# seqan/lambda

Hardware: AMD Instinct MI355X
Metric: GCUPS (gapped extension, full-rectangle parity mode; pass-1 cells per second of whole step) searchp BLOSUM62 (higher is better)
Workload: dtype f16x2 (exact small integers) + int32

## Files before the change

lambda_amd/csrc/lx_score_f16.hip:

```cpp
#include <hip/hip_runtime.h>

#include "lx_aids.h"
#include "lx_dp_common.h"

namespace lx
{

typedef _Float16 h2 __attribute__((ext_vector_type(2)));

#ifndef LX_F16_UNROLL
#define LX_F16_UNROLL 2
#endif
#ifndef LX_F16_CKPT_WAVES
#define LX_F16_CKPT_WAVES 3
#endif
#define LX_PRAGMA(x) _Pragma(#x)
#define LX_UNROLL(n) LX_PRAGMA(unroll n)

__device__ __forceinline__ h2 hmax3(h2 a, h2 b, h2 c)
{
    return __builtin_elementwise_maximum(__builtin_elementwise_maximum(a, b), c);
}
__device__ __forceinline__ h2 hmax(h2 a, h2 b)
{
    return __builtin_elementwise_maximum(a, b);
}
__device__ __forceinline__ h2 hsplat(float x)
{
    return h2{(_Float16)x, (_Float16)x};
}
__device__ __forceinline__ h2 as_h2(uint32_t x)
{
    return __builtin_bit_cast(h2, x);
}
__device__ __forceinline__ uint32_t as_u32(h2 x)
{
    return __builtin_bit_cast(uint32_t, x);
}

constexpr uint32_t kHalfNegInf2 = 0xfc00fc00u;

constexpr uint32_t kHalfTwoPowMinus24x2 = 0x00010001u;
__device__ __forceinline__ uint32_t c16_pack(h2 value_scaled, h2 diff_scaled)
{
    return (as_u32(diff_scaled) << 11) | as_u32(value_scaled);
}

template <int G, int C>
struct PairGeo
{
    static constexpr int kGroups   = 64 / G;
    static constexpr int kPanel    = G * C;
    static constexpr int kUsedDw   = (C + 1) / 2;
    static constexpr int kLaneDw   = (kUsedDw + 3) & ~3;
    static constexpr int kRowDw    = kLaneDw * G;
};

template <int G, int C, bool CKPT>
__global__ __launch_bounds__(64, (CKPT ? (C > 19 ? 2 : LX_F16_CKPT_WAVES) : 1)) void score_pair_kernel(ScoreParams p)
{
    static_assert(C <= 32, "profile rows hold 32 halves per lane");
    using Geo = PairGeo<G, C>;
    extern __shared__ uint32_t lds[];

    int const  lane     = threadIdx.x;
    int const  grp      = lane / G;
    int const  g        = lane % G;
    bool const is_first = (g == 0);

    uint64_t const pair   = (uint64_t)blockIdx.x * Geo::kGroups + grp;
    uint64_t const eA     = 2 * pair, eB = 2 * pair + 1;
    bool const     actA   = eA < p.n, actB = eB < p.n;

    ScoringDev const * __restrict__ sc = p.sc;
    int const      ge    = sc->ge;
    int const      nrows = p.nrows;
    uint32_t const padt  = (uint32_t)(nrows - 1);

    int             lq = 0, lsA = 0, lsB = 0;
    uint8_t const * q  = p.q_res;
    uint8_t const * sA = p.s_res;
    uint8_t const * sB = p.s_res;
    uint64_t        q_off = 0;
    if (actA)
    {
        Extension const x = p.ext[eA];
        lq    = (int)x.q_len;
        q_off = x.q_off;
        q += x.q_off;
        lsA = (int)x.s_len;
        if (lsA != 0)
            sA += x.s_off;
    }
    uint64_t q_offB = q_off;
    int      lqB    = lq;
    if (actB)
    {
        Extension const x = p.ext[eB];
        lqB    = (int)x.q_len;
        q_offB = x.q_off;
        lsB    = (int)x.s_len;
        if (lsB != 0)
            sB += x.s_off;
    }
    int const share_g = (p.pair_share > 0 && p.pair_share < Geo::kGroups) ? p.pair_share : Geo::kGroups;
    int const blk     = grp / share_g;
    {
        int const      leader = blk * share_g * G;
        uint64_t const q0     = ((uint64_t)(uint32_t)__shfl((int)(q_off >> 32), leader) << 32) | (uint32_t)__shfl((int)(uint32_t)q_off, leader);
        int const      l0     = __shfl(lq, leader);
        bool const     lead_in = __shfl(actA ? 1 : 0, leader) != 0;
        if (lead_in && ((actA && (q_off != q0 || lq != l0)) || (actB && (q_offB != q0 || lqB != l0))))
            atomicExch(p.err, 2);
    }

    int ls_max = max(lsA, lsB);
    int ls_min = min(actA ? lsA : 0x7fffffff, actB ? lsB : 0x7fffffff);
#pragma unroll
    for (int off = 32; off >= 1; off >>= 1)
    {
        ls_max = max(ls_max, __shfl_xor(ls_max, off));
        ls_min = min(ls_min, __shfl_xor(ls_min, off));
    }
    ls_max = __builtin_amdgcn_readfirstlane(ls_max);
    ls_min = __builtin_amdgcn_readfirstlane(ls_min);
    int const steps = (ls_max + G - 1 + 3) & ~3;

    int const col0  = g * C;
    int       bound = lq * sc->smax;
    if (__ballot(bound + (-ge) * (steps + G + 2) + sc->smax + 2 > 2046) != 0)
    {
        bound = 0;
#pragma unroll
        for (int c = 0; c < C; ++c)
        {
            int const j = col0 + c;
            if (j < lq)
                bound += sc->rowmax[q[j] & (kAlph - 1)];
        }
#pragma unroll
        for (int off = G / 2; off >= 1; off >>= 1)
            bound += __shfl_xor(bound, off);
    }
    bool too_big = __ballot((lq > Geo::kPanel) || (bound + (-ge) * (steps + G + 2) + sc->smax + 2 > 2046)) != 0;
    if constexpr (CKPT)
    {
        bool const broken = (__ballot(lq > Geo::kPanel) != 0) || (uint32_t)steps > p.steps_cap;
        if (broken && lane == 0)
            atomicExch(p.err, 3);
        too_big = too_big || broken;
    }

    if (too_big)
    {
        if (is_first)
        {
            if (actA)
                p.out_score[eA] = -1;
            if (actB)
                p.out_score[eB] = -1;
            if constexpr (CKPT)
            {
                EndCell none{};
                none.score = -1;
                if (actA)
                    p.ends[eA] = none;
                if (actB)
                    p.ends[eB] = none;
            }
        }
        return;
    }

    int const slot_dw = blk * (nrows * Geo::kRowDw);
    if (grp % share_g == 0)
    {
#pragma unroll 1
        for (int d = 0; d < Geo::kUsedDw; ++d)
        {
            uint32_t rows[2][16];
#pragma unroll
            for (int cc = 0; cc < 2; ++cc)
            {
                int const c  = 2 * d + cc;
                int const j  = col0 + c;
                uint32_t  ql = kAlph - 1;
                if (c < C && j < lq)
                    ql = q[j] & (kAlph - 1);
                uint4 const * mrow = reinterpret_cast<uint4 const *>(sc->mat_h + ql * kAlph);
#pragma unroll
                for (int x = 0; x < 4; ++x)
                {
                    uint4 const v      = mrow[x];
                    rows[cc][4 * x + 0] = v.x;
                    rows[cc][4 * x + 1] = v.y;
                    rows[cc][4 * x + 2] = v.z;
                    rows[cc][4 * x + 3] = v.w;
                }
            }
            uint32_t * dst = lds + slot_dw + g * Geo::kLaneDw + d;
#pragma unroll
            for (int w = 0; w < 16; ++w)
            {
                if (2 * w < nrows)
                {
                    dst[(2 * w) * Geo::kRowDw]     = __builtin_amdgcn_perm(rows[1][w], rows[0][w], 0x05040100u);
                    dst[(2 * w + 1) * Geo::kRowDw] = __builtin_amdgcn_perm(rows[1][w], rows[0][w], 0x07060302u);
                }
            }
        }
    }
    __builtin_amdgcn_fence(__ATOMIC_RELEASE, "wavefront");
    __builtin_amdgcn_wave_barrier();

    uint32_t const row_base  = (uint32_t)(slot_dw + g * Geo::kLaneDw) * 4u;
    constexpr uint32_t kRowBytes = Geo::kRowDw * 4;

    h2 const GE = hsplat((float)ge), G2 = hsplat((float)sc->g2), NGE = hsplat((float)-ge);
    h2       Z  = hsplat((float)(ge * g));
    h2       Hrow[C], F0[C];
#pragma unroll
    for (int c = 0; c < C; ++c)
    {
        Hrow[c] = Z + GE;
        F0[c]   = Z;
    }
    h2 diag0 = Z + GE;
    h2 sendH = Z + GE;
    h2 sendE = as_h2(kHalfNegInf2);
    h2 best  = hsplat(0.f);
    int      rowA = 0, rowB = 0;
    uint32_t tie  = 0;
    h2 const C24 = as_h2(kHalfTwoPowMinus24x2), NC24 = -C24, GEc = GE * C24;
    h2       nZc = -(Z * C24);
    h2       cmax = as_h2(kHalfNegInf2);
    using Lay = Ckpt16Layout<G, C>;
    constexpr uint32_t kW       = 2 * Geo::kGroups;
    constexpr bool     wslots   = CKPT;
    uint32_t * const   waveBase = CKPT ? p.ckpt + (uint64_t)blockIdx.x * kW * p.ckpt_stride : nullptr;
    uint32_t * const   slotA    = !CKPT ? nullptr : wslots ? waveBase + (2 * grp) * (G * 4) : p.ckpt + (actA ? eA : p.n) * p.ckpt_stride;
    uint32_t * const   slotB    = !CKPT ? nullptr : wslots ? waveBase + (2 * grp + 1) * (G * 4) : p.ckpt + (actB ? eB : p.n) * p.ckpt_stride;
    uint32_t const     octMul   = wslots ? kW * G : G;
    uint32_t const     ckMul    = (wslots ? kW * G : G) * (Lay::kCkDw / 4);
    uint32_t * const stage = lds + ((Geo::kGroups + share_g - 1) / share_g) * (nrows * Geo::kRowDw) + lane;

    auto step = [&](uint32_t tA, uint32_t tB, int slot8)
    {
        uint4 const * ra = reinterpret_cast<uint4 const *>(reinterpret_cast<char const *>(lds) + row_base + tA * kRowBytes);
        uint4 const * rb = reinterpret_cast<uint4 const *>(reinterpret_cast<char const *>(lds) + row_base + tB * kRowBytes);
        uint32_t      pa[Geo::kLaneDw], pb[Geo::kLaneDw];
#pragma unroll
        for (int x = 0; x < (Geo::kUsedDw + 3) / 4; ++x)
        {
            if (4 * x + 2 >= Geo::kUsedDw)
            {
                uint2 const va = *reinterpret_cast<uint2 const *>(ra + x), vb = *reinterpret_cast<uint2 const *>(rb + x);
                pa[4 * x] = va.x; pa[4 * x + 1] = va.y;
                pb[4 * x] = vb.x; pb[4 * x + 1] = vb.y;
            }
            else
            {
                uint4 const va = ra[x], vb = rb[x];
                pa[4 * x] = va.x; pa[4 * x + 1] = va.y; pa[4 * x + 2] = va.z; pa[4 * x + 3] = va.w;
                pb[4 * x] = vb.x; pb[4 * x + 1] = vb.y; pb[4 * x + 2] = vb.z; pb[4 * x + 3] = vb.w;
            }
        }

        h2 const recvH = as_h2((uint32_t)shift_from_left<G>((int)as_u32(sendH), (int)as_u32(Z), is_first));
        h2       Ecur  = as_h2((uint32_t)shift_from_left<G>((int)as_u32(sendE), (int)kHalfNegInf2, is_first));
        h2       dg    = diag0;
        diag0          = recvH;

        h2 const ZN     = Z + NGE;
        h2       rowmax = as_h2(kHalfNegInf2);
        h2       h      = Z;
#pragma unroll
        for (int c = 0; c < C; ++c)
        {
            uint32_t const sel = (c & 1) ? 0x07060302u : 0x05040100u;
            h2 const       sub = as_h2(__builtin_amdgcn_perm(pb[c >> 1], pa[c >> 1], sel));
            h2 const       tt  = dg + sub;
            dg                 = Hrow[c];
            h                  = hmax3(tt, Ecur, F0[c]);
            h2 const A         = h + G2;
            F0[c]              = hmax3(F0[c], A, ZN);
            Ecur               = hmax(Ecur, A) + GE;
            Hrow[c]            = h;
            if (c & 1)
                rowmax = hmax3(rowmax, Hrow[c - 1], h);
        }
        if (C & 1)
            rowmax = hmax(rowmax, h);
        sendH = h;
        sendE = Ecur;
        h2 const cand = rowmax - Z;
        if constexpr (CKPT)
        {
            cmax = hmax(cmax, cand);
            h2 const hc           = h * C24;
            stage[slot8 * 64]     = c16_pack(hc + nZc, __builtin_elementwise_fma(Ecur, NC24, hc));
            nZc                   = nZc + GEc;
        }
        else
            best = hmax(best, cand);
        Z = ZN;
    };
    auto flush_codes = [&](int k0)
    {
        if constexpr (CKPT)
        {
            uint32_t cw[8];
#pragma unroll
            for (int u = 0; u < 8; ++u)
                cw[u] = stage[u * 64];
            uint32_t const oi = ((uint32_t)k0 / 8) * octMul + (uint32_t)g;
            reinterpret_cast<uint4 *>(slotA)[oi] = make_uint4(__builtin_amdgcn_perm(cw[1], cw[0], 0x05040100u), __builtin_amdgcn_perm(cw[3], cw[2], 0x05040100u),
                                                              __builtin_amdgcn_perm(cw[5], cw[4], 0x05040100u), __builtin_amdgcn_perm(cw[7], cw[6], 0x05040100u));
            reinterpret_cast<uint4 *>(slotB)[oi] = make_uint4(__builtin_amdgcn_perm(cw[1], cw[0], 0x07060302u), __builtin_amdgcn_perm(cw[3], cw[2], 0x07060302u),
                                                              __builtin_amdgcn_perm(cw[5], cw[4], 0x07060302u), __builtin_amdgcn_perm(cw[7], cw[6], 0x07060302u));
        }
    };
    auto book = [&](int k0)
    {
        if constexpr (CKPT)
        {
            h2 const       nb   = hmax(best, cmax);
            uint32_t const rose = as_u32(nb) ^ as_u32(best), met = as_u32(cmax) ^ as_u32(best);
            bool const     gtA = (rose & 0xffffu) != 0, gtB = (rose >> 16) != 0;
            bool const     eqA = (met & 0xffffu) == 0, eqB = (met >> 16) == 0;
            int const last = k0 + 3 - g;
            rowA = gtA ? last : rowA;
            rowB = gtB ? last : rowB;
            tie  = (gtA ? (tie & ~1u) : (tie | (eqA ? 1u : 0u)));
            tie  = (gtB ? (tie & ~2u) : (tie | (eqB ? 2u : 0u)));
            best = nb;
            cmax = as_h2(kHalfNegInf2);
        }
    };
    auto chunk_done = [&](int k0)
    {
        if constexpr (CKPT)
        {
#ifndef LX_EXP_NO_FLUSH
            if (k0 & 4)
                flush_codes(k0);
#endif
        }
    };
    auto rowck_store = [&](int k0)
    {
        if constexpr (CKPT)
        {
            h2 const nzic = nZc - GEc, nGEc = -GEc;
            uint32_t code[2 * Lay::kCkDw];
#pragma unroll
            for (int c = 0; c < 2 * Lay::kCkDw; ++c)
                code[c] = c < C ? c16_pack(__builtin_elementwise_fma(Hrow[c < C ? c : 0], C24, nzic),
                                           __builtin_elementwise_fma(Hrow[c < C ? c : 0] - F0[c < C ? c : 0], C24, nGEc))
                                : 0u;
            uint32_t const base0 = (uint32_t)(Lay::bnd_dwords(p.steps_cap) / 4);
            uint4 * const  dA = wslots ? reinterpret_cast<uint4 *>(waveBase) + kW * base0 + (2 * grp) * (G * (Lay::kCkDw / 4)) : reinterpret_cast<uint4 *>(slotA) + base0;
            uint4 * const  dB = wslots ? reinterpret_cast<uint4 *>(waveBase) + kW * base0 + (2 * grp + 1) * (G * (Lay::kCkDw / 4)) : reinterpret_cast<uint4 *>(slotB) + base0;
#pragma unroll
            for (int x = 0; x < Lay::kCkDw / 4; ++x)
            {
                uint32_t wa[4], wb[4];
#pragma unroll
                for (int b = 0; b < 4; ++b)
                {
                    int const c = 2 * (4 * x + b);
                    wa[b]       = __builtin_amdgcn_perm(code[c + 1], code[c], 0x05040100u);
                    wb[b]       = __builtin_amdgcn_perm(code[c + 1], code[c], 0x07060302u);
                }
                uint32_t const qi = ((uint32_t)(k0 + 3) / 16) * ckMul + (uint32_t)g * (Lay::kCkDw / 4) + (uint32_t)x;
                dA[qi] = make_uint4(wa[0], wa[1], wa[2], wa[3]);
                dB[qi] = make_uint4(wb[0], wb[1], wb[2], wb[3]);
            }
        }
    };

    uint32_t const lscA = (uint32_t)max(lsA, 1) - 1u, lscB = (uint32_t)max(lsB, 1) - 1u;
    auto fetch_checked = [&](int k0, uint32_t (&ta)[4], uint32_t (&tb)[4])
    {
#pragma unroll
        for (int u = 0; u < 4; ++u)
        {
            uint32_t const i = (uint32_t)(k0 + u - g);
            ta[u]            = sA[min(i, lscA)];
            tb[u]            = sB[min(i, lscB)];
        }
    };
    auto mask_checked = [&](int k0, uint32_t (&ta)[4], uint32_t (&tb)[4])
    {
#pragma unroll
        for (int u = 0; u < 4; ++u)
        {
            uint32_t const i = (uint32_t)(k0 + u - g);
            ta[u]            = (i < (uint32_t)lsA) ? (ta[u] & (kAlph - 1)) : padt;
            tb[u]            = (i < (uint32_t)lsB) ? (tb[u] & (kAlph - 1)) : padt;
        }
    };

    int const steady_lo = (G - 1 + 3) & ~3;
    int const steady_hi = ls_min - 3;
    uint8_t const * spA = sA - g;
    uint8_t const * spB = sB - g;

    auto chunk_stores = [&](int k0)
    {
        chunk_done(k0);
        if (((k0 + 4) & 15) == 0)
        {
            book(k0);
#ifndef LX_EXP_NO_ROWCK
            rowck_store(k0);
#endif
        }
    };
    int      k0 = 0;
    uint32_t na[4], nb[4];
    fetch_checked(0, na, nb);
    while (k0 < steps)
    {
        bool const cur_steady = (k0 >= steady_lo) && (k0 < steady_hi);
        if (!cur_steady)
        {
            uint32_t ca[4] = {na[0], na[1], na[2], na[3]}, cb[4] = {nb[0], nb[1], nb[2], nb[3]};
            mask_checked(k0, ca, cb);
            fetch_checked(k0 + 4, na, nb);
#pragma unroll 1
            for (int u = 0; u < 4; ++u)
                step(ca[u], cb[u], (k0 & 4) + u);
            if constexpr (CKPT)
                asm volatile("" : "+v"(na[0]), "+v"(na[1]), "+v"(na[2]), "+v"(na[3]), "+v"(nb[0]), "+v"(nb[1]), "+v"(nb[2]), "+v"(nb[3])::"memory");
            chunk_stores(k0);
            k0 += 4;
        }
        else
        {
            uint32_t wa = *reinterpret_cast<unaligned_u32 const *>(spA + k0);
            uint32_t wb = *reinterpret_cast<unaligned_u32 const *>(spB + k0);
            if constexpr (CKPT)
                asm volatile("" : "+v"(wa), "+v"(wb)::"memory");
            while (k0 < steady_hi)
            {
                uint32_t const ca = wa, cb = wb;
                int const      kn = max(min(k0 + 4, ls_min - 4), 0);
                wa                = *reinterpret_cast<unaligned_u32 const *>(spA + kn);
                wb                = *reinterpret_cast<unaligned_u32 const *>(spB + kn);
LX_UNROLL(LX_F16_UNROLL)
                for (int u = 0; u < 4; ++u)
                    step((ca >> (8 * u)) & (kAlph - 1), (cb >> (8 * u)) & (kAlph - 1), (k0 & 4) + u);
                if constexpr (CKPT)
                    asm volatile("" : "+v"(wa), "+v"(wb)::"memory");
                chunk_stores(k0);
                k0 += 4;
            }
            fetch_checked(k0, na, nb);
        }
    }
    if (steps & 4)
        flush_codes(steps);
    if (steps & 15)
        book(steps - 4);

    if constexpr (!CKPT)
    {
#pragma unroll
        for (int off = G / 2; off >= 1; off >>= 1)
            best = hmax(best, as_h2((uint32_t)__shfl_xor((int)as_u32(best), off)));

        if (is_first)
        {
            if (actA)
                p.out_score[eA] = (int)(float)best.x;
            if (actB)
                p.out_score[eB] = (int)(float)best.y;
        }
    }
    else
    {
        auto finish = [&](int lbest, int lrow, int ltie, bool act, uint64_t e)
        {
            int gbest = lbest, gstrip = g, grow = lrow, gtie = ltie;
#pragma unroll
            for (int off = 1; off < G; off <<= 1)
            {
                int const  ob = __shfl_xor(gbest, off), os = __shfl_xor(gstrip, off), orow = __shfl_xor(grow, off), ot = __shfl_xor(gtie, off);
                bool const take = ob > gbest || (ob == gbest && os < gstrip);
                gbest  = take ? ob : gbest;
                gstrip = take ? os : gstrip;
                grow   = take ? orow : grow;
                gtie   = take ? ot : gtie;
            }
            if (is_first && act)
            {
                EndCell ec{};
                if (gbest > 0)
                {
                    ec.score = gbest;
                    ec.q_end = -(gstrip + 1);
                    ec.s_end = grow + 1;
                    ec.flags = (gtie ? kEndAmbiguous : 0) | kEndCompact | kEndWaveSlots;
                }
                p.ends[e]      = ec;
                p.out_score[e] = gbest;
            }
        };
        finish((int)(float)best.x, rowA, (int)(tie & 1u), actA, eA);
        finish((int)(float)best.y, rowB, (int)((tie >> 1) & 1u), actB, eB);
    }
}

template <int G, int C, bool CKPT = false>
static hipError_t launch_pair_cfg(ScoreParams const & p, hipStream_t stream)
{
    using Geo = PairGeo<G, C>;
    uint64_t const per_wave = 2ull * Geo::kGroups;
    uint64_t const blocks   = (p.n + per_wave - 1) / per_wave;
    if (blocks > 0x7fffffffull)
        return hipErrorInvalidValue;
    int const    slots = (p.pair_share > 0 && p.pair_share < Geo::kGroups) ? Geo::kGroups / p.pair_share : 1;
    if (slots * p.pair_share != Geo::kGroups && slots != 1)
        return hipErrorInvalidValue;
    size_t const lds = ((size_t)slots * (size_t)p.nrows * Geo::kRowDw + (CKPT ? 64 * 8 : 0)) * sizeof(uint32_t);
    hipLaunchKernelGGL((score_pair_kernel<G, C, CKPT>), dim3((unsigned)blocks), dim3(64), lds, stream, p);
    return hipGetLastError();
}

hipError_t launch_score_pair(int cfg, ScoreParams const & p, hipStream_t stream)
{
    if (p.n == 0)
        return hipSuccess;
    if (p.ckpt)
    {
        if (!p.ends || p.steps_cap % 16 != 0)
            return hipErrorInvalidValue;
        return cfg == 0   ? launch_pair_cfg<8, 19, true>(p, stream)
               : cfg == 5 ? launch_pair_cfg<16, 13, true>(p, stream)
               : cfg == 1 ? launch_pair_cfg<8, 13, true>(p, stream)
               : cfg == 7 ? launch_pair_cfg<8, 25, true>(p, stream)
                          : hipErrorInvalidValue;
    }
    switch (cfg)
    {
        case 0: return launch_pair_cfg<8, 19>(p, stream);
        case 1: return launch_pair_cfg<8, 13>(p, stream);
        case 2: return launch_pair_cfg<8, 16>(p, stream);
        case 3: return launch_pair_cfg<8, 8>(p, stream);
        case 4: return launch_pair_cfg<8, 24>(p, stream);
        case 5: return launch_pair_cfg<16, 13>(p, stream);
        case 6: return launch_pair_cfg<16, 10>(p, stream);
        case 7: return launch_pair_cfg<8, 25>(p, stream);
        default: return hipErrorInvalidValue;
    }
}

int score_pair_cfg_for(uint32_t max_qlen)
{
    if (max_qlen <= 64)
        return 3;
    if (max_qlen <= 104)
        return 1;
    if (max_qlen <= 128)
        return 2;
    if (max_qlen <= 152)
        return 0;
    if (max_qlen <= 192)
        return 4;
    if (max_qlen <= 200)
        return 7;
    if (max_qlen <= 208)
        return 5;
    return -1;
}

int score_pair_cfg_for_runs_of_8(uint32_t max_qlen)
{
    if (max_qlen <= 160)
        return 6;
    if (max_qlen <= 208)
        return 5;
    return -1;
}

int score_pair_cfg_cols(int cfg)
{
    static int const c[8] = {19, 13, 16, 8, 24, 13, 10, 25};
    return (cfg >= 0 && cfg < 8) ? c[cfg] : 0;
}

int score_pair_cfg_group(int cfg) { return (cfg == 5 || cfg == 6) ? 16 : 8; }

size_t score_pair_profile_bytes(int cfg, int nrows)
{
    int const G = score_pair_cfg_group(cfg), C = score_pair_cfg_cols(cfg);
    return (size_t)nrows * (size_t)((((C + 1) / 2 + 3) & ~3) * G) * sizeof(uint32_t);
}

}
```

Before: 5927.

## Interleave lane groups for DPP row shifts and share profile building across group

Remaps lanes so that for G=8 two groups interleave within each 16-lane DPP row. The left-neighbour H/E handoff can then use a single update_dpp row_shr instead of the shuffle-based shift_from_left, and reductions use strided xor shuffles. The LDS query-profile build is now split across all lanes of the sharing block rather than done by the leader group alone. This shortens the per-cell inner-loop dependency and the prologue, at the cost of more complex lane indexing. It risks subtle correctness issues in the handling of the boundary lane.

```diff
diff --git a/lambda_amd/csrc/lx_score_f16.hip b/lambda_amd/csrc/lx_score_f16.hip
--- a/lambda_amd/csrc/lx_score_f16.hip
+++ b/lambda_amd/csrc/lx_score_f16.hip
@@ -63,10 +63,14 @@
     using Geo = PairGeo<G, C>;
     extern __shared__ uint32_t lds[];
 
+    static_assert(G == 8 || G == 16, "lane groups of half a DPP row or a whole one");
+    constexpr int kGs     = G == 8 ? 2 : 1;
+    constexpr int kDppShr = 0x110 + kGs;
     int const  lane     = threadIdx.x;
-    int const  grp      = lane / G;
-    int const  g        = lane % G;
+    int const  g        = G == 8 ? (lane & 15) >> 1 : lane % G;
+    int const  grp      = G == 8 ? ((lane >> 4) << 1) | (lane & 1) : lane / G;
     bool const is_first = (g == 0);
+    auto lane_of = [](int group, int strip) { return G == 8 ? ((group >> 1) << 4) | (strip << 1) | (group & 1) : group * G + strip; };
 
     uint64_t const pair   = (uint64_t)blockIdx.x * Geo::kGroups + grp;
     uint64_t const eA     = 2 * pair, eB = 2 * pair + 1;
@@ -105,13 +109,17 @@
     }
     int const share_g = (p.pair_share > 0 && p.pair_share < Geo::kGroups) ? p.pair_share : Geo::kGroups;
     int const blk     = grp / share_g;
-    {
-        int const      leader = blk * share_g * G;
+    uint64_t  q_blk;
+    int       lq_blk;
+    {
+        int const      leader = lane_of(blk * share_g, 0);
         uint64_t const q0     = ((uint64_t)(uint32_t)__shfl((int)(q_off >> 32), leader) << 32) | (uint32_t)__shfl((int)(uint32_t)q_off, leader);
         int const      l0     = __shfl(lq, leader);
         bool const     lead_in = __shfl(actA ? 1 : 0, leader) != 0;
         if (lead_in && ((actA && (q_off != q0 || lq != l0)) || (actB && (q_offB != q0 || lqB != l0))))
             atomicExch(p.err, 2);
+        q_blk  = q0;
+        lq_blk = l0;
     }
 
     int ls_max = max(lsA, lsB);
@@ -140,7 +148,7 @@
         }
 #pragma unroll
         for (int off = G / 2; off >= 1; off >>= 1)
-            bound += __shfl_xor(bound, off);
+            bound += __shfl_xor(bound, off * kGs);
     }
     bool too_big = __ballot((lq > Geo::kPanel) || (bound + (-ge) * (steps + G + 2) + sc->smax + 2 > 2046)) != 0;
     if constexpr (CKPT)
@@ -173,39 +181,37 @@
     }
 
     int const slot_dw = blk * (nrows * Geo::kRowDw);
-    if (grp % share_g == 0)
-    {
+    {
+        constexpr int  kStripDw = G * Geo::kUsedDw;
+        int const      units    = ((nrows + 7) >> 3) * kStripDw;
+        int const      in_blk   = (grp - blk * share_g) * G + g;
+        uint8_t const * qb      = p.q_res + q_blk;
 #pragma unroll 1
-        for (int d = 0; d < Geo::kUsedDw; ++d)
-        {
-            uint32_t rows[2][16];
+        for (int u = in_blk; u < units; u += share_g * G)
+        {
+            int const x  = u / kStripDw;
+            int const sd = u - x * kStripDw;
+            int const sg = sd / Geo::kUsedDw, d = sd - sg * Geo::kUsedDw;
+            uint4     rows[2];
 #pragma unroll
             for (int cc = 0; cc < 2; ++cc)
             {
                 int const c  = 2 * d + cc;
-                int const j  = col0 + c;
+                int const j  = sg * C + c;
                 uint32_t  ql = kAlph - 1;
-                if (c < C && j < lq)
-                    ql = q[j] & (kAlph - 1);
-                uint4 const * mrow = reinterpret_cast<uint4 const *>(sc->mat_h + ql * kAlph);
-#pragma unroll
-                for (int x = 0; x < 4; ++x)
+                if (c < C && j < lq_blk)
+                    ql = qb[j] & (kAlph - 1);
+                rows[cc] = reinterpret_cast<uint4 const *>(sc->mat_h + ql * kAlph)[x];
+            }
+            uint32_t const r0[4] = {rows[0].x, rows[0].y, rows[0].z, rows[0].w}, r1[4] = {rows[1].x, rows[1].y, rows[1].z, rows[1].w};
+            uint32_t *     dst   = lds + slot_dw + (8 * x) * Geo::kRowDw + sg * Geo::kLaneDw + d;
+#pragma unroll
+            for (int w = 0; w < 4; ++w)
+            {
+                if (8 * x + 2 * w < nrows)
                 {
-                    uint4 const v      = mrow[x];
-                    rows[cc][4 * x + 0] = v.x;
-                    rows[cc][4 * x + 1] = v.y;
-                    rows[cc][4 * x + 2] = v.z;
-                    rows[cc][4 * x + 3] = v.w;
-                }
-            }
-            uint32_t * dst = lds + slot_dw + g * Geo::kLaneDw + d;
-#pragma unroll
-            for (int w = 0; w < 16; ++w)
-            {
-                if (2 * w < nrows)
-                {
-                    dst[(2 * w) * Geo::kRowDw]     = __builtin_amdgcn_perm(rows[1][w], rows[0][w], 0x05040100u);
-                    dst[(2 * w + 1) * Geo::kRowDw] = __builtin_amdgcn_perm(rows[1][w], rows[0][w], 0x07060302u);
+                    dst[(2 * w) * Geo::kRowDw]     = __builtin_amdgcn_perm(r1[w], r0[w], 0x05040100u);
+                    dst[(2 * w + 1) * Geo::kRowDw] = __builtin_amdgcn_perm(r1[w], r0[w], 0x07060302u);
                 }
             }
         }
@@ -228,6 +234,7 @@
     h2 diag0 = Z + GE;
     h2 sendH = Z + GE;
     h2 sendE = as_h2(kHalfNegInf2);
+    h2 recvE = as_h2(kHalfNegInf2);
     h2 best  = hsplat(0.f);
     int      rowA = 0, rowB = 0;
     uint32_t tie  = 0;
@@ -266,8 +273,9 @@
             }
         }
 
-        h2 const recvH = as_h2((uint32_t)shift_from_left<G>((int)as_u32(sendH), (int)as_u32(Z), is_first));
-        h2       Ecur  = as_h2((uint32_t)shift_from_left<G>((int)as_u32(sendE), (int)kHalfNegInf2, is_first));
+        h2 const recvH = as_h2((uint32_t)__builtin_amdgcn_update_dpp((int)as_u32(Z), (int)as_u32(sendH), kDppShr, 0xf, 0xf, false));
+        recvE          = as_h2((uint32_t)__builtin_amdgcn_update_dpp((int)as_u32(recvE), (int)as_u32(sendE), kDppShr, 0xf, 0xf, false));
+        h2       Ecur  = recvE;
         h2       dg    = diag0;
         diag0          = recvH;
 
@@ -468,7 +476,7 @@
     {
 #pragma unroll
         for (int off = G / 2; off >= 1; off >>= 1)
-            best = hmax(best, as_h2((uint32_t)__shfl_xor((int)as_u32(best), off)));
+            best = hmax(best, as_h2((uint32_t)__shfl_xor((int)as_u32(best), off * kGs)));
 
         if (is_first)
         {
@@ -486,7 +494,7 @@
 #pragma unroll
             for (int off = 1; off < G; off <<= 1)
             {
-                int const  ob = __shfl_xor(gbest, off), os = __shfl_xor(gstrip, off), orow = __shfl_xor(grow, off), ot = __shfl_xor(gtie, off);
+                int const  ob = __shfl_xor(gbest, off * kGs), os = __shfl_xor(gstrip, off * kGs), orow = __shfl_xor(grow, off * kGs), ot = __shfl_xor(gtie, off * kGs);
                 bool const take = ob > gbest || (ob == gbest && os < gstrip);
                 gbest  = take ? ob : gbest;
                 gstrip = take ? os : gstrip;
@@ -520,8 +528,9 @@
     uint64_t const blocks   = (p.n + per_wave - 1) / per_wave;
     if (blocks > 0x7fffffffull)
         return hipErrorInvalidValue;
-    int const    slots = (p.pair_share > 0 && p.pair_share < Geo::kGroups) ? Geo::kGroups / p.pair_share : 1;
-    if (slots * p.pair_share != Geo::kGroups && slots != 1)
+    bool const   split = p.pair_share > 0 && p.pair_share < Geo::kGroups;
+    int const    slots = split ? Geo::kGroups / p.pair_share : 1;
+    if (split && slots * p.pair_share != Geo::kGroups)
         return hipErrorInvalidValue;
     size_t const lds = ((size_t)slots * (size_t)p.nrows * Geo::kRowDw + (CKPT ? 64 * 8 : 0)) * sizeof(uint32_t);
     hipLaunchKernelGGL((score_pair_kernel<G, C, CKPT>), dim3((unsigned)blocks), dim3(64), lds, stream, p);
```

New measurement: 6043 (median of 6 runs). +2.0%, better.
